# burchim/AVEC

Hardware: AMD Instinct MI355X
Metric: AV utterances/sec fwd+bwd (audio T=400, video 100x88x88) (higher is better)
Workload: dtype bf16

## Files before the change

avec_amd/csrc/gemm.hip:

```cpp
#include "gemm_dev.h"

template <typename T, int BM, int BN, int MODE, bool SRC_F32, bool A16>
__global__ __launch_bounds__(256, 2) void gemm_nt_kernel(GemmArgs g) {
  constexpr int VEC = Elt<T>::VEC;
  constexpr int KE = BKB / (int)sizeof(T);
  constexpr int NCA = BM * 8 / 256, NCB = BN * 8 / 256;
  constexpr int MT = BM / 64, NT = BN / 64;
  constexpr int TILE = (BM + BN) * LDS_ROW;
  extern __shared__ __attribute__((aligned(16))) char smem[];
  const int tid = threadIdx.x, lane = tid & 63, wave = tid >> 6;
  const int wm = wave >> 1, wn = wave & 1;
  const long long m0 = (long long)blockIdx.x * BM; const int n0 = blockIdx.y * BN;
  const int kc = (tid & 7) * VEC;
  const int r0 = tid >> 3;

  RowInfo ra[NCA]; RowInfo rb[NCB];
  RowSrc ws; ws.ptr = g.W; ws.ld = g.ldw; ws.step = 0; ws.rows_out = ws.rows_in = 1;
#pragma unroll
  for (int i = 0; i < NCA; ++i) ra[i] = row_info<MODE>(g.a, m0 + r0 + i * 32, g.M);
#pragma unroll
  for (int i = 0; i < NCB; ++i) rb[i] = row_info<MODE_PLAIN>(ws, n0 + r0 + i * 32, g.N);

  f32x16 acc[MT][NT];
#pragma unroll
// ... 738 lines not shown
    for (int j = 0; j < NT; ++j)
#pragma unroll
      for (int r = 0; r < 16; ++r) acc[i][j][r] = 0.f;
  const int KT = (g.K + KE - 1) / KE;
  constexpr int LPT = NCA + NCB;
#define AVEC_WAIT_VM(n) asm volatile("s_waitcnt vmcnt(%0)" ::"n"(n) : "memory")
#pragma unroll
  for (int st = 0; st < STAGES - 1; ++st) if (st < KT) issue(st, st);
  for (int kt = 0; kt < KT; ++kt) {
    const int newer = min(STAGES - 2, KT - 1 - kt);
    if (STAGES <= 2 || newer <= 0) AVEC_WAIT_VM(0);
    else if (newer == 1) AVEC_WAIT_VM(LPT);
    else AVEC_WAIT_VM(2 * LPT);
    __builtin_amdgcn_s_barrier();
    asm volatile("" ::: "memory");
    if (kt + STAGES - 1 < KT) issue(kt + STAGES - 1, (kt + STAGES - 1) % STAGES);
    const char* As = smem + (kt % STAGES) * TILE; const char* Bs = As + BM * RB;
#pragma unroll
    for (int s2 = 0; s2 < 2; ++s2) {
      chunk16 fa[MT][2], fb[NT][2];
#pragma unroll
      for (int i = 0; i < MT; ++i)
#pragma unroll
        for (int h = 0; h < 2; ++h) fa[i][h] = *(const chunk16*)(As + offa[i] + (((4 * s2 + 2 * gsel + h) ^ swa[i]) << 4));
#pragma unroll
      for (int j = 0; j < NT; ++j)
#pragma unroll
        for (int h = 0; h < 2; ++h) fb[j][h] = *(const chunk16*)(Bs + offb[j] + (((4 * s2 + 2 * gsel + h) ^ swb[j]) << 4));
      asm volatile("" ::: "memory");
#pragma unroll
      for (int i = 0; i < MT; ++i) {
        const i32x8 a = {(int)fa[i][0].w[0], (int)fa[i][0].w[1], (int)fa[i][0].w[2], (int)fa[i][0].w[3], (int)fa[i][1].w[0], (int)fa[i][1].w[1], (int)fa[i][1].w[2], (int)fa[i][1].w[3]};
#pragma unroll
        for (int j = 0; j < NT; ++j) {
          const i32x8 b = {(int)fb[j][0].w[0], (int)fb[j][0].w[1], (int)fb[j][0].w[2], (int)fb[j][0].w[3], (int)fb[j][1].w[0], (int)fb[j][1].w[1], (int)fb[j][1].w[2], (int)fb[j][1].w[3]};
          acc[i][j] = __builtin_amdgcn_mfma_scale_f32_32x32x64_f8f6f4(a, b, acc[i][j], 0, 0, 0, 127, 0, 127);
        }
      }
    }
  }
#undef AVEC_WAIT_VM
  const float sc = (fmaxf(*amax_a, 1e-20f) * (1.0f / 448.0f)) * (fmaxf(*amax_w, 1e-20f) * (1.0f / 448.0f));
#pragma unroll
  for (int i = 0; i < MT; ++i)
#pragma unroll
    for (int j = 0; j < NT; ++j)
#pragma unroll
      for (int r = 0; r < 16; ++r) acc[i][j][r] *= sc;
  __syncthreads();
  nt_epilogue<T, BM, BN, MT, NT>(g, acc, smem, m0, n0, tid, lane, wm, wn);
}

struct TnArgs { const void* P; long long ldp; RowSrc q; float* O; void* Oact; long long ldo; long long M; int I, J, Iq, Jq; int m_per_block; float* pcs;
                int split, nb_inner, xcd_map, q_ohw, q_mg, q_nwrap; long long sPo, sPi, sQo, sQi, sOo, sOi; };

__device__ __forceinline__ int tn_swz(int col) { return (((col >> 2) ^ (col >> 3) ^ (col >> 4)) & 1) << 4; }

template <typename T>
__device__ __forceinline__ void store_transposed(char* S, int col0, int p, const chunk16& c0, const chunk16& c1) {
  constexpr int VEC = Elt<T>::VEC;
  if (sizeof(T) == 4) {
#pragma unroll
    for (int e = 0; e < VEC; ++e) *(uint32_t*)(S + (col0 + e) * LDS_ROW + ((p ^ tn_swz(col0 + e)) << 2)) = c0.w[e];
  } else {
#pragma unroll
    for (int e = 0; e < VEC; ++e) {
      const uint32_t w = (e & 1) ? __builtin_amdgcn_perm(c1.w[e >> 1], c0.w[e >> 1], 0x07060302u) : __builtin_amdgcn_perm(c1.w[e >> 1], c0.w[e >> 1], 0x05040100u);
      *(uint32_t*)(S + (col0 + e) * LDS_ROW + ((p ^ tn_swz(col0 + e)) << 2)) = w;
    }
  }
}

template <typename T, int BM, int BN, int MT, int NT>
__device__ __forceinline__ void mma_tile_swz(const char* As, const char* Bs, int wm, int wn, int lane, f32x16 (&acc)[MT][NT]) {
  int offa[MT], offb[NT], lowa[MT], lowb[NT];
#pragma unroll
  for (int i = 0; i < MT; ++i) { const int row = wm * (BM / 2) + i * 32 + (lane & 31); offa[i] = row * LDS_ROW; lowa[i] = ((lane >> 5) * 16) ^ (tn_swz(row) << 2); }
#pragma unroll
  for (int j = 0; j < NT; ++j) { const int row = wn * (BN / 2) + j * 32 + (lane & 31); offb[j] = row * LDS_ROW; lowb[j] = ((lane >> 5) * 16) ^ (tn_swz(row) << 2); }
#pragma unroll
  for (int kk = 0; kk < 4; ++kk) {
    chunk16 fa[MT], fb[NT];
#pragma unroll
    for (int i = 0; i < MT; ++i) fa[i] = *(const chunk16*)(As + offa[i] + (lowa[i] ^ (kk * 32)));
#pragma unroll
    for (int j = 0; j < NT; ++j) fb[j] = *(const chunk16*)(Bs + offb[j] + (lowb[j] ^ (kk * 32)));
#pragma unroll
    for (int i = 0; i < MT; ++i)
#pragma unroll
      for (int j = 0; j < NT; ++j) Mma<T>::run(fa[i], fb[j], acc[i][j]);
  }
}

template <typename T, int BI, int BJ, int MODE, bool Q_F32, bool A16>
__device__ __forceinline__ void gemm_tn_body(TnArgs g, const int bx, const int by, const int bz) {
  constexpr int VEC = Elt<T>::VEC;
  constexpr int RPT = sizeof(T) == 2 ? 2 : 1;
  constexpr int KE = 32 * RPT;
  constexpr int CPR_I = BI / VEC, CPR_J = BJ / VEC;
  constexpr int NTI = 32 * CPR_I / 256, NTJ = 32 * CPR_J / 256;
  constexpr int MT = BI / 64, NT = BJ / 64;
  constexpr int TILE = (BI + BJ) * LDS_ROW;
  constexpr bool Q_CONV = (MODE == MODE_CONV_FWD);
  extern __shared__ __attribute__((aligned(16))) char smem[];
  const int tid = threadIdx.x, lane = tid & 63, wave = tid >> 6;
  const int wm = wave >> 1, wn = wave & 1;
  const int i0 = bx * BI, j0 = by * BJ;
// ... 215 lines not shown
  }
  constexpr int CS_RF = 64 / (CPI * 4), CS_N = (KT / 4) / (4 * CS_RF);
  const bool do_cs = g.pcs != nullptr && by == 0;
  const int cs_pc = lane % CPI, cs_r4 = (lane / CPI) & 3, cs_rs = lane / (CPI * 4);
  float cs[8] = {0.f, 0.f, 0.f, 0.f, 0.f, 0.f, 0.f, 0.f};
  constexpr int LPT = NLI + NLJ;
#define AVEC_WAIT_VM(n) asm volatile("s_waitcnt vmcnt(%0)" ::"n"(n) : "memory")
  const int KTN = (int)((me - mb + KT - 1) / KT);
#pragma unroll
  for (int st = 0; st < STAGES - 1; ++st) if (st < KTN) issue(mb + (long long)st * KT, st);
  for (int kt = 0; kt < KTN; ++kt) {
    const int newer = min(STAGES - 2, KTN - 1 - kt);
    if (STAGES <= 2 || newer <= 0) AVEC_WAIT_VM(0);
    else if (newer == 1) AVEC_WAIT_VM(LPT);
    else AVEC_WAIT_VM(2 * LPT);
    __builtin_amdgcn_s_barrier();
    asm volatile("" ::: "memory");
    if (kt + STAGES - 1 < KTN) issue(mb + (long long)(kt + STAGES - 1) * KT, (kt + STAGES - 1) % STAGES);
    const char* S = smem + (kt % STAGES) * TILE;
    if (do_cs) {
#pragma unroll
      for (int n = 0; n < CS_N; ++n) {
        const int m = cs_r4 + 4 * (wave * CS_RF + cs_rs + 4 * CS_RF * n);
        const chunk16 c = *(const chunk16*)(S + m * (BI * 2) + (cs_pc << 4));
#pragma unroll
        for (int e = 0; e < 4; ++e) { cs[2 * e] += __uint_as_float(c.w[e] << 16); cs[2 * e + 1] += __uint_as_float(c.w[e] & 0xffff0000u); }
      }
    }
#pragma unroll
    for (int kk = 0; kk < KT / 16; ++kk) {
      chunk16 fa[MTI], fb[MTJ];
#pragma unroll
      for (int i = 0; i < MTI; ++i) fa[i] = tr_read8(S + offa[i][0] + kk * 16 * BI * 2, S + offa[i][1] + kk * 16 * BI * 2);
#pragma unroll
      for (int j = 0; j < MTJ; ++j) fb[j] = tr_read8(S + offb[j][0] + kk * 16 * BJ * 2, S + offb[j][1] + kk * 16 * BJ * 2);
#pragma unroll
      for (int i = 0; i < MTI; ++i)
#pragma unroll
        for (int j = 0; j < MTJ; ++j) Mma<T>::run(fa[i], fb[j], acc[i][j]);
    }
  }
#undef AVEC_WAIT_VM
  if (do_cs) {
    float* red = (float*)smem;
    __syncthreads();
    if (tid < BI) red[tid] = 0.f;
    __syncthreads();
    const int cl = (cs_pc ^ tr_swz<BI>(cs_r4)) << 3;
#pragma unroll
    for (int e = 0; e < 8; ++e) atomicAdd(red + cl + e, cs[e]);
    __syncthreads();
    if (tid < BI && i0 + tid < g.I) atomicAdd(g.pcs + i0 + tid, red[tid]);
  }
#pragma unroll
  for (int j = 0; j < MTJ; ++j) {
    const int col = j0 + wj * (BJ / 2) + j * 32 + (lane & 31);
    if (col >= g.J) continue;
#pragma unroll
    for (int i = 0; i < MTI; ++i)
#pragma unroll
      for (int r = 0; r < 16; ++r) {
        const int row = i0 + wi * (BI / 2) + i * 32 + (r & 3) + 8 * (r >> 2) + 4 * (lane >> 5);
        if (row < g.I) atomicAdd(Op + (long long)row * g.ldo + col, acc[i][j][r]);
      }
  }
}

template <int BI, int BJ, int MODE, int STAGES, bool Q32 = false, int KT = 64>
__global__ __launch_bounds__(256, 2) void gemm_tn_tr_kernel(TnArgs g) {
  if (g.xcd_map) {
    int l = xcd_logical(blockIdx.x + gridDim.x * (blockIdx.y + gridDim.y * blockIdx.z), gridDim.x * gridDim.y * gridDim.z);
    const int bx = l % gridDim.x; l /= gridDim.x;
    tn_tr_body<BI, BJ, MODE, STAGES, Q32, KT>(g, bx, l % gridDim.y, l / gridDim.y);
  } else tn_tr_body<BI, BJ, MODE, STAGES, Q32, KT>(g, blockIdx.x, blockIdx.y, blockIdx.z);
}

struct TnItem { const void* P; const void* Q; float* O; float* pcs; int ldp, ldq, ldo, M, I, J, Iq, Jq, m_per_block, split, gx, gy, rows_out, rows_in, step, first; };
struct TnGroup { TnItem it[AVEC_TN_GROUP_MAX]; int n, total, xcd_map; };
template <int BT, int STG = 2, int KT = 32>
__global__ __launch_bounds__(256, 2) void gemm_tn_tr_grouped_kernel(TnGroup grp) {
  const int w = grp.xcd_map ? xcd_logical(blockIdx.x, grp.total) : (int)blockIdx.x;
  int lo = 0, hi = grp.n - 1;
  while (lo < hi) { const int mid = (lo + hi + 1) >> 1; if (grp.it[mid].first <= w) lo = mid; else hi = mid - 1; }
  const TnItem& t = grp.it[lo];
  TnArgs g; g.P = t.P; g.ldp = t.ldp; g.q.ptr = t.Q; g.q.ld = t.ldq; g.q.rows_out = t.rows_out; g.q.rows_in = t.rows_in; g.q.step = t.step;
  g.q.H = g.q.W = g.q.C = g.q.KH = g.q.KW = g.q.stride = g.q.pad = g.q.OH = g.q.OW = 0;
  g.O = t.O; g.Oact = nullptr; g.ldo = t.ldo; g.M = t.M; g.I = t.I; g.J = t.J; g.Iq = t.Iq; g.Jq = t.Jq; g.m_per_block = t.m_per_block; g.pcs = t.pcs;
  g.split = t.split; g.nb_inner = 1; g.xcd_map = 0; g.q_ohw = 1; g.q_mg = 0; g.q_nwrap = 0; g.sPo = g.sPi = g.sQo = g.sQi = g.sOo = g.sOi = 0;
  int l = w - t.first; const int bx = l % t.gx; l /= t.gx; const int by = l % t.gy; const int bz = l / t.gy;
  tn_tr_body<BT, BT, MODE_PLAIN, STG, false, KT>(g, bx, by, bz);
}

#include <stdint.h>
#include <stdlib.h>
#include <string.h>
static RowSrc make_src(const void* ptr, const avec_rows_t* d) {
  RowSrc s; s.ptr = ptr; s.ld = d->ld; s.rows_out = d->rows_out; s.rows_in = d->rows_in; s.step = d->step;
  s.H = d->H; s.W = d->W; s.C = d->C; s.KH = d->KH; s.KW = d->KW; s.stride = d->stride; s.pad = d->pad; s.OH = d->OH; s.OW = d->OW;
  return s;
}

template <typename K> static int want_lds(K kern, size_t bytes) {
  static const void* done[256]; static int ndone = 0;
  for (int i = 0; i < ndone; ++i) if (done[i] == (const void*)kern) return 0;
  hipError_t e = hipFuncSetAttribute((const void*)kern, hipFuncAttributeMaxDynamicSharedMemorySize, (int)bytes);
  if (e != hipSuccess) { avec_set_error("hipFuncSetAttribute failed: %s", hipGetErrorString(e)); return (int)e; }
  if (ndone < 256) done[ndone++] = (const void*)kern;
  return 0;
}

static bool aligned16(const void* p) { return (((uintptr_t)p) & 15) == 0; }
static bool epi_tr_ok(const GemmArgs& g) {
  static const bool off = getenv("AVEC_NO_EPI_TR") != nullptr;
  const Epi& e = g.e;
  return !off && !e.out_f32 && !e.out_pre && !e.bias && e.act == 0 && !(e.drop_p > 0.f) && !e.dact && !e.colsum && !e.bnb_y && g.N % 8 == 0 &&
         e.ldo % 8 == 0 && aligned16(e.out) && (!e.res || (e.res_act && e.ldres % 8 == 0 && aligned16(e.res)));
}

static bool plain_tr_ok(const GemmArgs& g) {
  static const bool off = getenv("AVEC_NO_PLAIN_TR") != nullptr || getenv("AVEC_NO_EPI_TR") != nullptr;
  const Epi& e = g.e;
  const long long ob = e.out_f32 ? 4 : 2;
  return !off && !e.colsum && !e.stats && !e.bnb_y && g.N % 8 == 0 && g.N >= 8 && aligned16(e.out) && (e.ldo * ob) % 16 == 0 &&
         (!e.out_pre || (aligned16(e.out_pre) && e.ldpre % 8 == 0)) && (!e.bias || aligned16(e.bias)) && (!e.dact || (aligned16(e.dact_z) && e.ldz % 8 == 0)) &&
         (!e.res || (aligned16(e.res) && (e.ldres * (e.res_act ? 2 : 4)) % 16 == 0));
}

template <typename T, int BM, int BN>
static int launch_nt_mode(const GemmArgs& g_in, int mode, int src_f32, hipStream_t st) {
  GemmArgs g = g_in;
  dim3 grid((unsigned)((g.M + BM - 1) / BM), (unsigned)((g.N + BN - 1) / BN));
  size_t lds = (size_t)2 * (BM + BN) * LDS_ROW;
  constexpr int VEC = Elt<T>::VEC;
  const bool f32src = src_f32 && sizeof(T) == 2;
  const bool a16 = aligned16(g.a.ptr) && aligned16(g.W) && g.K % VEC == 0 && g.ldw % VEC == 0 &&
                   (mode != MODE_PLAIN || (g.a.ld % (f32src ? 4 : VEC) == 0));
  static const bool use_glds_ = true;
  static const bool no_ktail = false;
  const bool plain_any = sizeof(T) == 2 && mode == MODE_PLAIN && !f32src && use_glds_ && !no_ktail && (g.K % 8 == 0 || g.K % 8 == 4) && g.K >= 8 && g.ldw >= g.K && g.a.ld >= g.K &&
                         g.a.step <= 1;
  g.ktail = (plain_any && g.K % 8 == 4) ? 4 : 0;
// ... 147 lines not shown
    static const bool no_perm = getenv("AVEC_NO_PERM2") != nullptr;
    if (!no_perm && dtype == AVEC_BF16 && g.fast_conv && a_mode == MODE_CONV_BWD && a_rows->stride == 2 && M == imgs * (long long)a_rows->H * a_rows->W) {
      g.perm2 = 1; g.pImgs = imgs;
    }
  }
  Epi& e = g.e;
  e.out = ep->out; e.ldo = ep->ldo; e.out_f32 = ep->out_f32; e.out_pre = ep->out_pre; e.ldpre = ep->ldpre; e.bias = ep->bias;
  e.act = ep->act; e.drop_p = ep->drop_p; e.rng = (const unsigned long long*)ep->rng; e.stream = ep->rng_stream;
  e.res = ep->res; e.ldres = ep->ldres; e.alpha = ep->alpha; e.res_act = ep->res_act; e.dact_z = ep->dact_z; e.ldz = ep->ldz; e.dact = ep->dact;
  e.colsum = ep->colsum; e.stats = ep->stats;
  e.bnb_y = ep->bnb_y; e.ldby = ep->ldby; e.bnb_ss = ep->bnb_ss; e.bnb_mask = ep->bnb_mask; e.res_cls0 = ep->res_cls0; e.res_mask = ep->res_mask;
  AVEC_CHECK_ARG(!e.res_mask || (dtype == AVEC_BF16 && !a_f32 && a_mode != AVEC_ROWS_PLAIN && e.res && e.res_act && !e.res_cls0 && e.ldres % 8 == 0),
                 "gemm_nt: res_mask needs a bf16 convolution product with a bf16 residual whose rows are whole 8-element pieces");
  AVEC_CHECK_ARG(!e.res_cls0 || (g.perm2 && e.res), "gemm_nt: res_cls0 needs a bf16 stride-2 backward-data product that runs in parity-class order");
  AVEC_CHECK_ARG(!e.bnb_y || (e.stats && N % 4 == 0 && !(e.ldo & 3) && !(e.ldby & 3) && !(e.ldres & 3) && !(e.ldz & 3) && !(e.ldpre & 3) && (!e.bnb_mask || e.bnb_ss) && (e.bnb_mask || e.dact == 2 || e.dact == 0)),
                 "gemm_nt: the BatchNorm-backward fusion needs stats, N %% 4 == 0 and row strides that are multiples of 4");
  AVEC_CHECK_ARG(!(e.drop_p > 0.f) || e.rng, "gemm_nt: dropout without rng state");
  int r = 1;
  if (dtype == AVEC_BF16 && !a_f32 && a_mode != AVEC_ROWS_PLAIN) r = launch_conv_shift(g, a_mode, stream);
  if (r == 1 && dtype == AVEC_BF16 && !a_f32 && a_mode != AVEC_ROWS_PLAIN) r = avec_launch_conv_s2(g, a_mode, stream);
  if (r == 1) r = (dtype == AVEC_BF16) ? launch_nt<bf16>(g, a_mode, a_f32, stream) : launch_nt<float>(g, a_mode, a_f32, stream);
  if (r) return r;
  AVEC_LAUNCH_CHECK();
  return 0;
}


extern "C" int avec_gemm_nt_fp8(const void* A, long long lda, const void* W, long long ldw, long long M, int N, int K,
                                const float* amax_a, const float* amax_w, const avec_epilogue_t* ep, hipStream_t stream) {
  AVEC_CHECK_ARG(A && W && ep && ep->out && amax_a && amax_w, "gemm_nt_fp8: null pointer");
  AVEC_CHECK_ARG(M > 0 && N > 0 && K > 0 && K % 16 == 0 && lda % 16 == 0 && ldw % 16 == 0 && aligned16(A) && aligned16(W),
                 "gemm_nt_fp8: M=%lld N=%d K=%d lda=%lld ldw=%lld: K and the row strides must be multiples of 16 bytes, operands 16-byte aligned", M, N, K, lda, ldw);
  GemmArgs g; memset(&g, 0, sizeof(g));
  g.a.ptr = A; g.a.ld = lda; g.W = W; g.ldw = ldw; g.M = M; g.N = N; g.K = K;
  Epi& e = g.e;
  e.out = ep->out; e.ldo = ep->ldo; e.out_f32 = ep->out_f32; e.out_pre = ep->out_pre; e.ldpre = ep->ldpre; e.bias = ep->bias;
  e.act = ep->act; e.drop_p = ep->drop_p; e.rng = (const unsigned long long*)ep->rng; e.stream = ep->rng_stream;
  e.res = ep->res; e.ldres = ep->ldres; e.alpha = ep->alpha; e.res_act = ep->res_act; e.dact_z = ep->dact_z; e.ldz = ep->ldz; e.dact = ep->dact;
  e.colsum = ep->colsum; e.stats = ep->stats;
  AVEC_CHECK_ARG(!(e.drop_p > 0.f) || e.rng, "gemm_nt_fp8: dropout without rng state");
#define F8(BM, BN, S_) do { dim3 grid((unsigned)((M + BM - 1) / BM), (unsigned)((N + BN - 1) / BN)); \
    const size_t ring = (size_t)S_ * (BM + BN) * 128, epi = (size_t)64 * (BN + 4) * 4 + 10 * BN * 4; const size_t lds = ring > epi ? ring : epi; \
    if (int r = want_lds(gemm_nt_fp8_kernel<BM, BN, S_>, lds)) return r; \
    hipLaunchKernelGGL((gemm_nt_fp8_kernel<BM, BN, S_>), grid, dim3(256), lds, stream, g, amax_a, amax_w); } while (0)
  const long long t128 = ((M + 127) / 128) * ((N + 127) / 128);
  if (N > 64 && t128 >= 384) F8(128, 128, 2);
  else if (((M + 127) / 128) * ((N + 63) / 64) >= 384) F8(128, 64, 2);
  else F8(64, 64, 4);
#undef F8
  AVEC_LAUNCH_CHECK();
  return 0;
}

static thread_local TnMulti* tn_collect = nullptr;
template <typename T, int BI, int BJ>
static int launch_tn_tile(TnArgs g, int mode, int q_f32, int nbatch, hipStream_t st) {
  constexpr int KE = BKB / (int)sizeof(T);
  int tiles = ((g.I + BI - 1) / BI) * ((g.J + BJ - 1) / BJ) * nbatch;
  long long ksteps = (g.M + KE - 1) / KE;
  static const long long wg_env = getenv("AVEC_TN_WGS") ? atoll(getenv("AVEC_TN_WGS")) : 0;
  const long long wg_target = wg_env > 0 ? wg_env : (mode != MODE_PLAIN ? 896 : 512);
  long long split = (wg_target + tiles - 1) / tiles; if (split > ksteps / 4) split = ksteps / 4; if (split < 1 || g.Oact) split = 1;
  long long per = ((ksteps + split - 1) / split) * KE;
  split = (g.M + per - 1) / per;
  g.m_per_block = (int)per; g.split = (int)split;
  dim3 grid((g.I + BI - 1) / BI, (g.J + BJ - 1) / BJ, (unsigned)(split * nbatch));
  size_t lds = (size_t)2 * (BI + BJ) * LDS_ROW;
  constexpr int VEC = Elt<T>::VEC;
  const bool f32src = q_f32 && sizeof(T) == 2;
  const bool a16 = nbatch == 1 && aligned16(g.P) && aligned16(g.q.ptr) && g.Iq % VEC == 0 && g.Jq % VEC == 0 && g.ldp % VEC == 0 &&
                   (mode != MODE_PLAIN || (g.q.ld % (f32src ? 4 : VEC) == 0));
  if (sizeof(T) == 2 && a16 && !f32src && !g.Oact && (mode == MODE_PLAIN || g.q_mg != 0)) {
    static const bool use_tr = true;
    if (use_tr) {
      static const int kt_env = getenv("AVEC_TN_KT") ? atoi(getenv("AVEC_TN_KT")) : 32;
      const long long q_elems = mode == MODE_PLAIN ? 0 : ((g.M + (long long)g.q.OH * g.q.OW - 1) / ((long long)g.q.OH * g.q.OW) + 1) * g.q.H * g.q.W * g.q.C;
      const bool q32 = q_elems < (1ll << 31);
#define LT(MODE, Q32, KT_) do { const size_t l2 = (size_t)2 * KT_ * (BI + BJ) * 2; g.q_nwrap = (KT_ + g.q_ohw - 1) / g.q_ohw; avec_note_kernel("gemm_tn_tr_kernel<%d,%d,%d,2,%d,%d>", BI, BJ, MODE, (int)Q32, KT_); if (int r = want_lds(gemm_tn_tr_kernel<BI, BJ, MODE, 2, Q32, KT_>, l2)) return r; \
        hipLaunchKernelGGL((gemm_tn_tr_kernel<BI, BJ, MODE, 2, Q32, KT_>), grid, dim3(256), l2, st, g); return 0; } while (0)
#define LK(KT_) do { if (mode == MODE_PLAIN) LT(MODE_PLAIN, false, KT_); else if (q32) LT(MODE_CONV_FWD, true, KT_); else LT(MODE_CONV_FWD, false, KT_); } while (0)
      if (kt_env == 64) LK(64); else LK(32);
#undef LK
#undef LT
    }
  }
  if (g.pcs) {
    static const bool side_wgrad = false;
    if (int r = colsum_launch(sizeof(T) == 2 ? AVEC_BF16 : AVEC_F32, g.P, g.ldp, g.pcs, g.M, g.I, !side_wgrad, st)) return r;
  }
#define L(MODE, F, A) do { avec_note_kernel("gemm_tn_kernel<%s,%d,%d,%d,%d,%d>", (sizeof(T) == 2 ? "bf16" : "float"), BI, BJ, MODE, (int)F, (int)A); if (int r = want_lds(gemm_tn_kernel<T, BI, BJ, MODE, F, A>, lds)) return r; hipLaunchKernelGGL((gemm_tn_kernel<T, BI, BJ, MODE, F, A>), grid, dim3(256), lds, st, g); } while (0)
  if (tn_collect && sizeof(T) == 2 && BI == 64 && BJ == 64 && mode == MODE_PLAIN && !f32src && !a16 && !g.pcs && tn_collect->n < AVEC_TN_MULTI_MAX) {
    TnMulti& m = *tn_collect; const int k = m.n++;
    m.g[k] = g; m.gx[k] = (int)grid.x; m.gy[k] = (int)grid.y; m.first[k + 1] = m.first[k] + (int)(grid.x * grid.y * grid.z);
    return 0;
  }
  if (mode == MODE_PLAIN) {
    if (f32src) { if (a16) L(MODE_PLAIN, true, true); else L(MODE_PLAIN, true, false); }
    else { if (a16) L(MODE_PLAIN, false, true); else L(MODE_PLAIN, false, false); }
  } else { if (a16) L(MODE_CONV_FWD, false, true); else L(MODE_CONV_FWD, false, false); }
#undef L
  return 0;
}

static int gemm_tn_impl(int dtype, const void* P, long long ldp, const void* Q, const avec_rows_t* q_rows, int q_mode, int q_f32,
                        float* O, void* Oact, long long ldo, long long M, int I, int J, int nb_outer, int nb_inner, const long long* strides, float* p_colsum, hipStream_t stream) {
  AVEC_CHECK_ARG(dtype == AVEC_F32 || dtype == AVEC_BF16, "gemm_tn: bad dtype %d", dtype);
  AVEC_CHECK_ARG(P && Q && (O || Oact) && q_rows, "gemm_tn: null pointer");
  AVEC_CHECK_ARG(M > 0 && I > 0 && J > 0 && nb_outer > 0 && nb_inner > 0, "gemm_tn: bad dims");
  AVEC_CHECK_ARG(q_mode == MODE_PLAIN || q_mode == MODE_CONV_FWD, "gemm_tn: bad q_mode %d", q_mode);
  const int vec = dtype == AVEC_BF16 ? 8 : 4;
  const int Jq = (q_mode == MODE_PLAIN && q_rows->ld >= (J + vec - 1) / vec * vec) ? (J + vec - 1) / vec * vec : J;
  const int Iq = (ldp >= (I + vec - 1) / vec * vec) ? (I + vec - 1) / vec * vec : I;
  AVEC_CHECK_ARG(Iq >= vec && Jq >= vec && (dtype == AVEC_F32 || (Iq % 2 == 0 && Jq % 2 == 0 && ldp % 2 == 0)), "gemm_tn: I=%d, J=%d: need >= %d and (bf16) even I, J, ldp", I, J, vec);
  AVEC_CHECK_ARG(q_mode != MODE_PLAIN || dtype == AVEC_F32 || q_rows->ld % 2 == 0, "gemm_tn: ldq must be even");
  AVEC_CHECK_ARG(q_mode == MODE_PLAIN || q_rows->C % vec == 0, "gemm_tn: conv C=%d must be a multiple of %d", q_rows->C, vec);
  AVEC_CHECK_ARG(!(q_f32 && dtype == AVEC_BF16) || Jq % 4 == 0, "gemm_tn: fp32-source staging needs J %% 4 == 0");
  TnArgs g; g.P = P; g.ldp = ldp; g.q = make_src(Q, q_rows); g.O = O; g.Oact = Oact; g.ldo = ldo; g.M = M; g.I = I; g.J = J; g.Iq = Iq; g.Jq = Jq; g.m_per_block = 0; g.pcs = p_colsum;
  g.split = 1; g.nb_inner = nb_inner;
  g.q_ohw = 1; g.q_mg = 0; g.q_nwrap = 0;
  if (q_mode != MODE_PLAIN && q_rows->OW > 0 && q_rows->OH > 0 && (long long)q_rows->OH * q_rows->OW <= 4096) {
    const int ohw = q_rows->OH * q_rows->OW; const unsigned mg = ((1u << 20) + (unsigned)q_rows->OW - 1u) / (unsigned)q_rows->OW;
    bool exact = true; for (int px = 0; px < ohw && exact; ++px) exact = (int)(((unsigned)px * mg) >> 20) == px / q_rows->OW;
    g.q_ohw = ohw; g.q_mg = exact ? (int)mg : 0;
  }
  { static const bool no_xcd = false; g.xcd_map = no_xcd ? 0 : 1; }
  g.sPo = strides ? strides[0] : 0; g.sPi = strides ? strides[1] : 0; g.sQo = strides ? strides[2] : 0; g.sQi = strides ? strides[3] : 0;
  g.sOo = strides ? strides[4] : 0; g.sOi = strides ? strides[5] : 0;
  if (dtype == AVEC_BF16 && strides) for (int i = 0; i < 2; ++i) AVEC_CHECK_ARG(strides[i] % 2 == 0, "gemm_tn: bf16 batch strides of P must be even");
  const int nbatch = nb_outer * nb_inner;
  bool big = (I >= 128 && J >= 128) && ((long long)((I + 127) / 128) * ((J + 127) / 128) * nbatch >= 48 || M >= 32768);
  int r;
  const bool wide = !big && I <= 64 && J >= 128 && M >= 32768 && dtype == AVEC_BF16 && !q_f32 && nbatch == 1 && aligned16(P) && aligned16(Q) && Iq % 8 == 0 && Jq % 8 == 0 &&
                    ldp % 8 == 0 && (q_mode != MODE_PLAIN || q_rows->ld % 8 == 0);
  if (dtype == AVEC_BF16) r = big ? launch_tn_tile<bf16, 128, 128>(g, q_mode, q_f32, nbatch, stream) : wide ? launch_tn_tile<bf16, 64, 128>(g, q_mode, q_f32, nbatch, stream)
                                                                                                    : launch_tn_tile<bf16, 64, 64>(g, q_mode, q_f32, nbatch, stream);
  else r = big ? launch_tn_tile<float, 128, 128>(g, q_mode, q_f32, nbatch, stream) : launch_tn_tile<float, 64, 64>(g, q_mode, q_f32, nbatch, stream);
  if (r) return r;
  AVEC_LAUNCH_CHECK();
  return 0;
}

extern "C" int avec_gemm_tn(int dtype, const void* P, long long ldp, const void* Q, const avec_rows_t* q_rows, int q_mode, int q_f32,
                            float* O, long long ldo, long long M, int I, int J, hipStream_t stream) {
  return gemm_tn_impl(dtype, P, ldp, Q, q_rows, q_mode, q_f32, O, nullptr, ldo, M, I, J, 1, 1, nullptr, nullptr, stream);
}
extern "C" int avec_gemm_tn_bias(int dtype, const void* P, long long ldp, const void* Q, const avec_rows_t* q_rows, int q_mode, int q_f32,
                                 float* O, long long ldo, float* p_colsum, long long M, int I, int J, hipStream_t stream) {
  AVEC_CHECK_ARG(!p_colsum || (I % 4 == 0 && ldp % 4 == 0), "gemm_tn_bias: column sums need I %% 4 == 0 and ldp %% 4 == 0");
  return gemm_tn_impl(dtype, P, ldp, Q, q_rows, q_mode, q_f32, O, nullptr, ldo, M, I, J, 1, 1, nullptr, p_colsum, stream);
}

extern "C" int avec_gemm_tn_batched(int dtype, const void* P, long long ldp, const void* Q, long long ldq, float* O, long long ldo, long long M, int I, int J,
                                    int nb_outer, int nb_inner, const long long* strides6, hipStream_t stream) {
  avec_rows_t rows = {}; rows.ld = ldq;
  AVEC_CHECK_ARG(strides6, "gemm_tn_batched: null strides");
  return gemm_tn_impl(dtype, P, ldp, Q, &rows, MODE_PLAIN, 0, O, nullptr, ldo, M, I, J, nb_outer, nb_inner, strides6, nullptr, stream);
}
extern "C" int avec_gemm_tn_batched_store(int dtype, const void* P, long long ldp, const void* Q, long long ldq, void* O_act, long long ldo, long long M, int I, int J,
                                          int nb_outer, int nb_inner, const long long* strides6, hipStream_t stream) {
  avec_rows_t rows = {}; rows.ld = ldq;
  AVEC_CHECK_ARG(strides6 && O_act, "gemm_tn_batched_store: null pointer");
  return gemm_tn_impl(dtype, P, ldp, Q, &rows, MODE_PLAIN, 0, nullptr, O_act, ldo, M, I, J, nb_outer, nb_inner, strides6, nullptr, stream);
}

extern "C" int avec_gemm_tn_batched_multi(int dtype, const avec_tn_batched_t* items, int n, hipStream_t stream) {
  AVEC_CHECK_ARG(items && n >= 1 && n <= AVEC_TN_MULTI_MAX, "gemm_tn_batched_multi: need 1..%d problems (got %d)", AVEC_TN_MULTI_MAX, n);
  static const bool off = false;
  TnMulti m; m.n = 0; m.first[0] = 0;
  if (!off) tn_collect = &m;
  int rc = 0;
  for (int k = 0; k < n && rc == 0; ++k) {
    const avec_tn_batched_t& t = items[k];
    avec_rows_t rows = {}; rows.ld = t.ldq;
    if (!t.strides6 || (!t.O && !t.O_act)) { avec_set_error("gemm_tn_batched_multi: problem %d: null pointer", k); rc = -1; break; }
    rc = gemm_tn_impl(dtype, t.P, t.ldp, t.Q, &rows, MODE_PLAIN, 0, t.O_act ? nullptr : t.O, t.O_act, t.ldo, t.M, t.I, t.J, t.nb_outer, t.nb_inner, t.strides6, nullptr, stream);
  }
  tn_collect = nullptr;
  if (rc) return rc;
  if (m.n > 0) {
    const size_t lds = (size_t)2 * (64 + 64) * LDS_ROW;
    avec_note_kernel("gemm_tn_multi_kernel<%d>", m.n);
    if (int r = want_lds(gemm_tn_multi_kernel, lds)) return r;
    hipLaunchKernelGGL(gemm_tn_multi_kernel, dim3((unsigned)m.first[m.n]), dim3(256), lds, stream, m);
    AVEC_LAUNCH_CHECK();
  }
  return 0;
}

static bool tn_item_ok(int dtype, const avec_tn_item_t& t) {
  if (dtype != AVEC_BF16 || !t.P || !t.Q || !t.O || t.M <= 0 || t.I <= 0 || t.J <= 0) return false;
  if (t.ldp < t.I || t.ldq < t.J) return false;
  if (t.p_colsum && (t.I % 4 || t.ldp % 4)) return false;
  return t.M < (1ll << 31) && t.ldp < (1ll << 31) && t.ldq < (1ll << 31) && t.ldo < (1ll << 31);
}
extern "C" int avec_gemm_tn_grouped_ok(int dtype, const avec_tn_item_t* item) { return item && tn_item_ok(dtype, *item) ? 1 : 0; }

extern "C" int avec_gemm_tn_grouped(int dtype, const avec_tn_item_t* items, int n, hipStream_t stream) {
  AVEC_CHECK_ARG(items && n > 0 && n <= AVEC_TN_GROUP_MAX, "gemm_tn_grouped: need 1..%d items (got %d)", AVEC_TN_GROUP_MAX, n);
  for (int k = 0; k < n; ++k) AVEC_CHECK_ARG(tn_item_ok(dtype, items[k]), "gemm_tn_grouped: item %d is not eligible (bf16 operands, row strides >= widths, bias sums need I %% 4 == 0)", k);
  static const int bt_env = 0;
  long long t128 = 0;
  for (int k = 0; k < n; ++k) t128 += (long long)((items[k].I + 127) / 128) * ((items[k].J + 127) / 128);
  const int BT = bt_env == 64 || bt_env == 128 ? bt_env : (t128 >= 96 ? 128 : 64);
  static const long long wg_env = 0;
  const long long wg_target = wg_env > 0 ? wg_env : 512;
  long long per = 256;
  for (long long cand = 8192; cand >= 256; cand -= 64) {
    long long wgs = 0;
    for (int k = 0; k < n; ++k) wgs += (long long)((items[k].I + BT - 1) / BT) * ((items[k].J + BT - 1) / BT) * ((items[k].M + cand - 1) / cand);
    if (wgs >= wg_target) { per = cand; break; }
  }
  TnGroup grp; grp.n = n;
  int first = 0;
  for (int k = 0; k < n; ++k) {
    const avec_tn_item_t& s = items[k]; TnItem& t = grp.it[k];
    t.P = s.P; t.Q = s.Q; t.O = s.O; t.pcs = s.p_colsum; t.ldp = (int)s.ldp; t.ldq = (int)s.ldq; t.ldo = (int)s.ldo; t.M = (int)s.M; t.I = s.I; t.J = s.J;
    t.Iq = (s.I + 7) / 8 * 8; t.Jq = (s.J + 7) / 8 * 8;
    t.rows_out = s.q_rows_out > 0 ? s.q_rows_out : 1; t.rows_in = s.q_rows_in > 0 ? s.q_rows_in : 1; t.step = s.q_step;
    long long mp = per; if (mp > s.M) mp = (s.M + 63) / 64 * 64;
    t.m_per_block = (int)mp; t.split = (int)((s.M + mp - 1) / mp);
    t.gx = (s.I + BT - 1) / BT; t.gy = (s.J + BT - 1) / BT; t.first = first;
    first += t.gx * t.gy * t.split;
  }
  grp.total = first;
  static const bool no_xcd = false;
  grp.xcd_map = no_xcd ? 0 : 1;
  static const int kt_env = 64;
  static const int stg_env = 2;
  const int KT = kt_env == 32 ? 32 : 64, STG = (stg_env == 4 && KT == 32) ? 4 : 2;
  const size_t lds = (size_t)STG * KT * (BT + BT) * 2;
  avec_note_kernel("gemm_tn_tr_grouped_kernel<%d,%d,%d>", BT, STG, KT);
#define TNG(BT_, S_, K_) do { if (BT == BT_ && STG == S_ && KT == K_) { if (int r = want_lds(gemm_tn_tr_grouped_kernel<BT_, S_, K_>, lds)) return r; \
    hipLaunchKernelGGL((gemm_tn_tr_grouped_kernel<BT_, S_, K_>), dim3((unsigned)first), dim3(256), lds, stream, grp); } } while (0)
  TNG(128, 2, 32); TNG(128, 2, 64); TNG(64, 2, 32); TNG(64, 2, 64); TNG(128, 4, 32); TNG(64, 4, 32);
#undef TNG
  AVEC_LAUNCH_CHECK();
  return 0;
}
```

avec_amd/csrc/vec.h:

```cpp
#pragma once
#include "common.h"
#include <cstdlib>

template <typename T> __device__ __forceinline__ void ld4(const T* p, float v[4]);
template <> __device__ __forceinline__ void ld4<float>(const float* p, float v[4]) { float4 t = *(const float4*)p; v[0] = t.x; v[1] = t.y; v[2] = t.z; v[3] = t.w; }
template <> __device__ __forceinline__ void ld4<bf16>(const bf16* p, float v[4]) {
  uint2 t = *(const uint2*)p;
  v[0] = __uint_as_float(t.x << 16); v[1] = __uint_as_float(t.x & 0xffff0000u);
  v[2] = __uint_as_float(t.y << 16); v[3] = __uint_as_float(t.y & 0xffff0000u);
}
template <typename T> __device__ __forceinline__ void st4(T* p, const float v[4]);
template <> __device__ __forceinline__ void st4<float>(float* p, const float v[4]) { *(float4*)p = make_float4(v[0], v[1], v[2], v[3]); }
template <> __device__ __forceinline__ void st4<bf16>(bf16* p, const float v[4]) {
  uint2 t; t.x = f32x2_to_bf16x2(v[0], v[1]);
  t.y = f32x2_to_bf16x2(v[2], v[3]);
  *(uint2*)p = t;
}

template <typename T> __device__ __forceinline__ void ld8(const T* p, float v[8]);
template <> __device__ __forceinline__ void ld8<float>(const float* p, float v[8]) { ld4<float>(p, v); ld4<float>(p + 4, v + 4); }
template <> __device__ __forceinline__ void ld8<bf16>(const bf16* p, float v[8]) {
  uint4 t = *(const uint4*)p; const uint32_t w[4] = {t.x, t.y, t.z, t.w};
#pragma unroll
  for (int k = 0; k < 4; ++k) { v[2 * k] = __uint_as_float(w[k] << 16); v[2 * k + 1] = __uint_as_float(w[k] & 0xffff0000u); }
}
template <typename T> __device__ __forceinline__ void st8(T* p, const float v[8]);
template <> __device__ __forceinline__ void st8<float>(float* p, const float v[8]) { st4<float>(p, v); st4<float>(p + 4, v + 4); }
template <> __device__ __forceinline__ void st8<bf16>(bf16* p, const float v[8]) {
  uint4 t;
  t.x = f32x2_to_bf16x2(v[0], v[1]); t.y = f32x2_to_bf16x2(v[2], v[3]);
  t.z = f32x2_to_bf16x2(v[4], v[5]); t.w = f32x2_to_bf16x2(v[6], v[7]);
  *(uint4*)p = t;
}

__device__ __forceinline__ void bf8_to_f32(const uint4& t, float v[8]) {
  const uint32_t w[4] = {t.x, t.y, t.z, t.w};
#pragma unroll
  for (int k = 0; k < 4; ++k) { v[2 * k] = __uint_as_float(w[k] << 16); v[2 * k + 1] = __uint_as_float(w[k] & 0xffff0000u); }
}
template <typename T> struct Raw8;
template <> struct Raw8<bf16> { uint4 t; __device__ __forceinline__ void load(const bf16* p) { t = *(const uint4*)p; } __device__ __forceinline__ void get(float v[8]) const { bf8_to_f32(t, v); } };
template <> struct Raw8<float> { float4 a, b; __device__ __forceinline__ void load(const float* p) { a = *(const float4*)p; b = *(const float4*)(p + 4); }
  __device__ __forceinline__ void get(float v[8]) const { v[0] = a.x; v[1] = a.y; v[2] = a.z; v[3] = a.w; v[4] = b.x; v[5] = b.y; v[6] = b.z; v[7] = b.w; } };
#define DISPATCH_T(dtype, ...) do { if ((dtype) == AVEC_BF16) { typedef bf16 T; __VA_ARGS__; } else { typedef float T; __VA_ARGS__; } } while (0)


struct ColWs { float* partial; };
ColWs avec_reduce_ws(size_t partial_floats, hipStream_t st);

__device__ __forceinline__ float* ws_slot(const ColWs& ws, unsigned colblock, unsigned slot, unsigned nslots, int ncols) {
  return ws.partial + ((size_t)colblock * nslots + slot) * ncols;
}
static constexpr int FIN_MAXNV = 20;
struct ColFin { const float* partial; float* dst[FIN_MAXNV]; int NV, W, C, nslots, dstride; };
__global__ __launch_bounds__(256) void col_finalize_kernel(ColFin f);
int colsum_launch(int dtype, const void* x, long long ld, float* out, long long M, int N, bool use_ws, hipStream_t st);
int col_finalize(const ColWs& ws, unsigned colblocks, unsigned nslots, int NV, int W, float* const* dst, int C, hipStream_t st, int dstride = 1);

template <int NV>
__device__ __forceinline__ void colreduce_atomic(float (&part)[NV][4], float* const (&dst)[NV], int col, int C, const ColWs& ws = ColWs{nullptr}) {
  __shared__ float red[8][32][4];
  const int tx = threadIdx.x & 31, ty = threadIdx.x >> 5;
  float* mine = ws.partial ? ws_slot(ws, blockIdx.x, blockIdx.y, gridDim.y, NV * 128) : nullptr;
#pragma unroll
  for (int n = 0; n < NV; ++n) {
    for (int e = 0; e < 4; ++e) red[ty][tx][e] = part[n][e];
    __syncthreads();
    if (ty == 0) {
      for (int e = 0; e < 4; ++e) {
        float s = 0.f;
        for (int y = 0; y < 8; ++y) s += red[y][tx][e];
        if (mine) mine[n * 128 + tx * 4 + e] = s;
        else if (col + e < C && dst[n]) atomicAdd(dst[n] + col + e, s);
      }
    }
    __syncthreads();
  }
}
static inline ColWs col_ws(dim3 grid, int NV, hipStream_t st) { return avec_reduce_ws((size_t)grid.x * grid.y * NV * 128, st); }
static inline long long col_ws_min_atomics() { return 16384; }
static inline ColWs col_ws_if(dim3 grid, int NV, int C, hipStream_t st) {
  const long long atomics = (long long)grid.y * NV * C;
  return atomics > col_ws_min_atomics() ? col_ws(grid, NV, st) : ColWs{nullptr};
}

static inline dim3 col_grid(long long M, int C) {
  unsigned gx = (unsigned)((C / 4 + 31) / 32);
  long long gy = (M + 63) / 64; long long cap = 2048 / gx; if (cap < 1) cap = 1; if (gy > cap) gy = cap; if (gy < 1) gy = 1;
  return dim3(gx, (unsigned)gy);
}

struct Col8 { int L, R, r, l; bool active; };
__device__ __forceinline__ Col8 col8_map(int C) {
  Col8 m; m.L = C >> 3; m.R = 256 / m.L; m.r = threadIdx.x / m.L; m.l = threadIdx.x - m.r * m.L; m.active = m.r < m.R; return m;
}
template <int NV>
__device__ __forceinline__ void colreduce8_atomic(float (&part)[NV][8], float* const (&dst)[NV], const Col8& m, const ColWs& ws = ColWs{nullptr}) {
  __shared__ float red8[NV * 8][256];
#pragma unroll
  for (int n = 0; n < NV; ++n)
#pragma unroll
    for (int e = 0; e < 8; ++e) red8[n * 8 + e][threadIdx.x] = m.active ? part[n][e] : 0.f;
  __syncthreads();
  const int C = m.L * 8;
  float* mine = ws.partial ? ws_slot(ws, 0, blockIdx.x, gridDim.x, NV * C) : nullptr;
  for (int o = threadIdx.x; o < NV * 8 * m.L; o += 256) {
    const int q = o / m.L, l = o - q * m.L; float s = 0.f;
    for (int rr = 0; rr < m.R; ++rr) s += red8[q][rr * m.L + l];
    if (mine) mine[(q >> 3) * C + l * 8 + (q & 7)] = s;
    else {
// ... 21 lines not shown
```

Measured before the change: 1844.

## Replace split-K atomic accumulation in TN weight-grad GEMMs with slab reduction

Split-K partial tiles from the TN (weight-gradient) GEMM kernels are now written to a workspace slab instead of being atomically added to the output. A new grouped tile-slab-sum kernel then reduces the partials deterministically and adds them into the output. Grouped items with no split and no output overlap get plain read-modify-write stores instead of atomics. The aim is to cut float atomic contention on output tiles, at the cost of extra workspace traffic and one more kernel launch.

Result: no change. 1829 (-0.8%).

```diff
diff --git a/avec_amd/csrc/gemm.hip b/avec_amd/csrc/gemm.hip
--- a/avec_amd/csrc/gemm.hip
+++ b/avec_amd/csrc/gemm.hip
@@ -814,7 +814,8 @@
 }
 
 struct TnArgs { const void* P; long long ldp; RowSrc q; float* O; void* Oact; long long ldo; long long M; int I, J, Iq, Jq; int m_per_block; float* pcs;
-                int split, nb_inner, xcd_map, q_ohw, q_mg, q_nwrap; long long sPo, sPi, sQo, sQi, sOo, sOi; };
+                int split, nb_inner, xcd_map, q_ohw, q_mg, q_nwrap; long long sPo, sPi, sQo, sQi, sOo, sOi;
+                float* slab; int slab_gx, own; };
 
 __device__ __forceinline__ int tn_swz(int col) { return (((col >> 2) ^ (col >> 3) ^ (col >> 4)) & 1) << 4; }
 
@@ -1136,6 +1137,17 @@
     __syncthreads();
     if (tid < BI && i0 + tid < g.I) atomicAdd(g.pcs + i0 + tid, red[tid]);
   }
+  if (g.slab) {
+    float* sp = g.slab + ((long long)(by * g.slab_gx + bx) * g.split + zs) * (BI * BJ) + wave * (MTI * MTJ * 1024) + lane * 4;
+#pragma unroll
+    for (int i = 0; i < MTI; ++i)
+#pragma unroll
+      for (int j = 0; j < MTJ; ++j)
+#pragma unroll
+        for (int q = 0; q < 4; ++q)
+          *(float4*)(sp + ((i * MTJ + j) * 4 + q) * 256) = make_float4(acc[i][j][4 * q], acc[i][j][4 * q + 1], acc[i][j][4 * q + 2], acc[i][j][4 * q + 3]);
+    return;
+  }
 #pragma unroll
   for (int j = 0; j < MTJ; ++j) {
     const int col = j0 + wj * (BJ / 2) + j * 32 + (lane & 31);
@@ -1145,9 +1157,43 @@
 #pragma unroll
       for (int r = 0; r < 16; ++r) {
         const int row = i0 + wi * (BI / 2) + i * 32 + (r & 3) + 8 * (r >> 2) + 4 * (lane >> 5);
-        if (row < g.I) atomicAdd(Op + (long long)row * g.ldo + col, acc[i][j][r]);
-      }
-  }
+        if (row < g.I) { float* o = Op + (long long)row * g.ldo + col; if (g.own) *o += acc[i][j][r]; else atomicAdd(o, acc[i][j][r]); }
+      }
+  }
+}
+
+__global__ __launch_bounds__(256) void tn_slab_sum_kernel(TsGroup grp) {
+  __shared__ float4 red[256];
+  const int w = blockIdx.x, tid = threadIdx.x;
+  int lo = 0, hi = grp.n - 1;
+  while (lo < hi) { const int mid = (lo + hi + 1) >> 1; if (grp.it[mid].first <= w) lo = mid; else hi = mid - 1; }
+  const TsItem& t = grp.it[lo];
+  const int BI = grp.BI, BJ = grp.BJ, sg = grp.sg, LP = 256 / sg, tile4 = BI * BJ / 4, CH = tile4 / LP;
+  const int l = w - t.first, tile = l / CH, idx4 = (l - tile * CH) * LP + (tid % LP), cls = tid / LP;
+  const float* sp = grp.slab + ((long long)t.tile0 + (long long)tile * t.split) * (BI * BJ) + idx4 * 4;
+  float4 a = make_float4(0.f, 0.f, 0.f, 0.f);
+  int s = cls;
+  for (; s + 3 * sg < t.split; s += 4 * sg) {
+    const float4 v0 = *(const float4*)(sp + (long long)s * (BI * BJ)), v1 = *(const float4*)(sp + (long long)(s + sg) * (BI * BJ));
+    const float4 v2 = *(const float4*)(sp + (long long)(s + 2 * sg) * (BI * BJ)), v3 = *(const float4*)(sp + (long long)(s + 3 * sg) * (BI * BJ));
+    a.x = (((a.x + v0.x) + v1.x) + v2.x) + v3.x; a.y = (((a.y + v0.y) + v1.y) + v2.y) + v3.y; a.z = (((a.z + v0.z) + v1.z) + v2.z) + v3.z; a.w = (((a.w + v0.w) + v1.w) + v2.w) + v3.w;
+  }
+  for (; s < t.split; s += sg) { const float4 v = *(const float4*)(sp + (long long)s * (BI * BJ)); a.x += v.x; a.y += v.y; a.z += v.z; a.w += v.w; }
+  if (sg > 1) {
+    red[tid] = a;
+    __syncthreads();
+    if (cls != 0) return;
+    for (int c = 1; c < sg; ++c) { const float4 v = red[c * LP + tid]; a.x += v.x; a.y += v.y; a.z += v.z; a.w += v.w; }
+  }
+  const int MTI = BI / 64, MTJ = BJ / 64, lane = idx4 & 63, q = (idx4 >> 6) & 3;
+  int u = idx4 >> 8; const int j = u % MTJ; u /= MTJ; const int i = u % MTI, wave = u / MTI;
+  const int bx = tile % t.gx, by = tile / t.gx;
+  const int row = bx * BI + (wave >> 1) * (BI / 2) + i * 32 + 8 * q + 4 * (lane >> 5), col = by * BJ + (wave & 1) * (BJ / 2) + j * 32 + (lane & 31);
+  if (col >= t.J) return;
+  float* o = t.O + (long long)row * t.ldo + col;
+  const float v[4] = {a.x, a.y, a.z, a.w};
+#pragma unroll
+  for (int e = 0; e < 4; ++e) if (row + e < t.I) o[(long long)e * t.ldo] += v[e];
 }
 
 template <int BI, int BJ, int MODE, int STAGES, bool Q32 = false, int KT = 64>
@@ -1159,8 +1205,8 @@
   } else tn_tr_body<BI, BJ, MODE, STAGES, Q32, KT>(g, blockIdx.x, blockIdx.y, blockIdx.z);
 }
 
-struct TnItem { const void* P; const void* Q; float* O; float* pcs; int ldp, ldq, ldo, M, I, J, Iq, Jq, m_per_block, split, gx, gy, rows_out, rows_in, step, first; };
-struct TnGroup { TnItem it[AVEC_TN_GROUP_MAX]; int n, total, xcd_map; };
+struct TnItem { const void* P; const void* Q; float* O; float* pcs; int ldp, ldq, ldo, M, I, J, Iq, Jq, m_per_block, split, gx, gy, rows_out, rows_in, step, first, slab0, own; };
+struct TnGroup { TnItem it[AVEC_TN_GROUP_MAX]; float* slab; int n, total, xcd_map; };
 template <int BT, int STG = 2, int KT = 32>
 __global__ __launch_bounds__(256, 2) void gemm_tn_tr_grouped_kernel(TnGroup grp) {
   const int w = grp.xcd_map ? xcd_logical(blockIdx.x, grp.total) : (int)blockIdx.x;
@@ -1171,6 +1217,7 @@
   g.q.H = g.q.W = g.q.C = g.q.KH = g.q.KW = g.q.stride = g.q.pad = g.q.OH = g.q.OW = 0;
   g.O = t.O; g.Oact = nullptr; g.ldo = t.ldo; g.M = t.M; g.I = t.I; g.J = t.J; g.Iq = t.Iq; g.Jq = t.Jq; g.m_per_block = t.m_per_block; g.pcs = t.pcs;
   g.split = t.split; g.nb_inner = 1; g.xcd_map = 0; g.q_ohw = 1; g.q_mg = 0; g.q_nwrap = 0; g.sPo = g.sPi = g.sQo = g.sQi = g.sOo = g.sOi = 0;
+  g.slab = t.slab0 >= 0 ? grp.slab + (long long)t.slab0 * (BT * BT) : nullptr; g.slab_gx = t.gx; g.own = t.own;
   int l = w - t.first; const int bx = l % t.gx; l /= t.gx; const int by = l % t.gy; const int bz = l / t.gy;
   tn_tr_body<BT, BT, MODE_PLAIN, STG, false, KT>(g, bx, by, bz);
 }
@@ -1424,6 +1471,19 @@
   return 0;
 }
 
+static int tn_slabs_on() { static const int on = getenv("AVEC_TN_SLABS") ? atoi(getenv("AVEC_TN_SLABS")) : 7; return on; }
+static int g_tn_last[4];
+extern "C" int avec_tn_last_launch(int* out4) { for (int i = 0; i < 4; ++i) out4[i] = g_tn_last[i]; return 0; }
+int tile_slab_sum(TsGroup& grp, hipStream_t st) {
+  int smax = 1, first = 0;
+  for (int k = 0; k < grp.n; ++k) if (grp.it[k].split > smax) smax = grp.it[k].split;
+  grp.sg = smax >= 16 ? 4 : 1;
+  const int ch = grp.BI * grp.BJ / 4 / (256 / grp.sg);
+  for (int k = 0; k < grp.n; ++k) { TsItem& t = grp.it[k]; t.first = first; first += t.gx * ((t.J + grp.BJ - 1) / grp.BJ) * ch; }
+  hipLaunchKernelGGL(tn_slab_sum_kernel, dim3((unsigned)first), dim3(256), 0, st, grp);
+  return 0;
+}
+
 static thread_local TnMulti* tn_collect = nullptr;
 template <typename T, int BI, int BJ>
 static int launch_tn_tile(TnArgs g, int mode, int q_f32, int nbatch, hipStream_t st) {
@@ -1448,8 +1508,18 @@
       static const int kt_env = getenv("AVEC_TN_KT") ? atoi(getenv("AVEC_TN_KT")) : 32;
       const long long q_elems = mode == MODE_PLAIN ? 0 : ((g.M + (long long)g.q.OH * g.q.OW - 1) / ((long long)g.q.OH * g.q.OW) + 1) * g.q.H * g.q.W * g.q.C;
       const bool q32 = q_elems < (1ll << 31);
+      TsGroup ts; ts.n = 0;
+      if (split > 1 && nbatch == 1 && (tn_slabs_on() & 4)) {
+        const ColWs ws = avec_reduce_ws((size_t)tiles * (size_t)split * BI * BJ, st);
+        if (ws.partial) {
+          g.slab = ws.partial; g.slab_gx = (int)grid.x;
+          ts.n = 1; ts.slab = ws.partial; ts.BI = BI; ts.BJ = BJ;
+          TsItem& t = ts.it[0]; t.O = g.O; t.ldo = (int)g.ldo; t.I = g.I; t.J = g.J; t.gx = (int)grid.x; t.split = (int)split; t.tile0 = 0;
+        }
+      }
+      g_tn_last[0] = (int)split; g_tn_last[1] = ts.n; g_tn_last[2] = 0; g_tn_last[3] = 1 - ts.n;
 #define LT(MODE, Q32, KT_) do { const size_t l2 = (size_t)2 * KT_ * (BI + BJ) * 2; g.q_nwrap = (KT_ + g.q_ohw - 1) / g.q_ohw; avec_note_kernel("gemm_tn_tr_kernel<%d,%d,%d,2,%d,%d>", BI, BJ, MODE, (int)Q32, KT_); if (int r = want_lds(gemm_tn_tr_kernel<BI, BJ, MODE, 2, Q32, KT_>, l2)) return r; \
-        hipLaunchKernelGGL((gemm_tn_tr_kernel<BI, BJ, MODE, 2, Q32, KT_>), grid, dim3(256), l2, st, g); return 0; } while (0)
+        hipLaunchKernelGGL((gemm_tn_tr_kernel<BI, BJ, MODE, 2, Q32, KT_>), grid, dim3(256), l2, st, g); return ts.n ? tile_slab_sum(ts, st) : 0; } while (0)
 #define LK(KT_) do { if (mode == MODE_PLAIN) LT(MODE_PLAIN, false, KT_); else if (q32) LT(MODE_CONV_FWD, true, KT_); else LT(MODE_CONV_FWD, false, KT_); } while (0)
       if (kt_env == 64) LK(64); else LK(32);
 #undef LK
@@ -1488,7 +1558,7 @@
   AVEC_CHECK_ARG(q_mode == MODE_PLAIN || q_rows->C % vec == 0, "gemm_tn: conv C=%d must be a multiple of %d", q_rows->C, vec);
   AVEC_CHECK_ARG(!(q_f32 && dtype == AVEC_BF16) || Jq % 4 == 0, "gemm_tn: fp32-source staging needs J %% 4 == 0");
   TnArgs g; g.P = P; g.ldp = ldp; g.q = make_src(Q, q_rows); g.O = O; g.Oact = Oact; g.ldo = ldo; g.M = M; g.I = I; g.J = J; g.Iq = Iq; g.Jq = Jq; g.m_per_block = 0; g.pcs = p_colsum;
-  g.split = 1; g.nb_inner = nb_inner;
+  g.split = 1; g.nb_inner = nb_inner; g.slab = nullptr; g.slab_gx = 0; g.own = 0;
   g.q_ohw = 1; g.q_mg = 0; g.q_nwrap = 0;
   if (q_mode != MODE_PLAIN && q_rows->OW > 0 && q_rows->OH > 0 && (long long)q_rows->OH * q_rows->OW <= 4096) {
     const int ohw = q_rows->OH * q_rows->OW; const unsigned mg = ((1u << 20) + (unsigned)q_rows->OW - 1u) / (unsigned)q_rows->OW;
@@ -1574,7 +1644,7 @@
   long long t128 = 0;
   for (int k = 0; k < n; ++k) t128 += (long long)((items[k].I + 127) / 128) * ((items[k].J + 127) / 128);
   const int BT = bt_env == 64 || bt_env == 128 ? bt_env : (t128 >= 96 ? 128 : 64);
-  static const long long wg_env = 0;
+  static const long long wg_env = getenv("AVEC_TNG_WGS") ? atoll(getenv("AVEC_TNG_WGS")) : 0;
   const long long wg_target = wg_env > 0 ? wg_env : 512;
   long long per = 256;
   for (long long cand = 8192; cand >= 256; cand -= 64) {
@@ -1591,10 +1661,32 @@
     t.rows_out = s.q_rows_out > 0 ? s.q_rows_out : 1; t.rows_in = s.q_rows_in > 0 ? s.q_rows_in : 1; t.step = s.q_step;
     long long mp = per; if (mp > s.M) mp = (s.M + 63) / 64 * 64;
     t.m_per_block = (int)mp; t.split = (int)((s.M + mp - 1) / mp);
-    t.gx = (s.I + BT - 1) / BT; t.gy = (s.J + BT - 1) / BT; t.first = first;
+    t.gx = (s.I + BT - 1) / BT; t.gy = (s.J + BT - 1) / BT; t.first = first; t.slab0 = -1; t.own = 0;
     first += t.gx * t.gy * t.split;
   }
-  grp.total = first;
+  grp.total = first; grp.slab = nullptr;
+  TsGroup ts; ts.n = 0; ts.BI = ts.BJ = BT;
+  int smax = 1, n_own = 0;
+  if (tn_slabs_on()) {
+    long long slabs = 0;
+    for (int k = 0; k < n; ++k) {
+      TnItem& t = grp.it[k]; if (t.split > smax) smax = t.split;
+      const float* lo = t.O; const float* hi = t.O + (long long)(t.I - 1) * t.ldo + t.J;
+      bool alone = true;
+      for (int m = 0; m < n && alone; ++m) if (m != k) { const TnItem& u = grp.it[m]; alone = !(u.O < hi && lo < u.O + (long long)(u.I - 1) * u.ldo + u.J); }
+      if (!alone) continue;
+      if (t.split == 1) { if (tn_slabs_on() & 2) { t.own = 1; ++n_own; } }
+      else if (tn_slabs_on() & 1) { t.slab0 = (int)slabs; slabs += (long long)t.gx * t.gy * t.split; }
+    }
+    const ColWs ws = slabs > 0 && slabs < (1 << 24) ? avec_reduce_ws((size_t)slabs * BT * BT, stream) : ColWs{nullptr};
+    for (int k = 0; k < n; ++k) {
+      TnItem& t = grp.it[k]; if (t.slab0 < 0) continue;
+      if (!ws.partial) { t.slab0 = -1; continue; }
+      TsItem& q = ts.it[ts.n++]; q.O = t.O; q.ldo = t.ldo; q.I = t.I; q.J = t.J; q.gx = t.gx; q.split = t.split; q.tile0 = t.slab0;
+    }
+    grp.slab = ws.partial; ts.slab = ws.partial;
+  }
+  g_tn_last[0] = smax; g_tn_last[1] = ts.n; g_tn_last[2] = n_own; g_tn_last[3] = n - ts.n - n_own;
   static const bool no_xcd = false;
   grp.xcd_map = no_xcd ? 0 : 1;
   static const int kt_env = 64;
@@ -1606,6 +1698,7 @@
     hipLaunchKernelGGL((gemm_tn_tr_grouped_kernel<BT_, S_, K_>), dim3((unsigned)first), dim3(256), lds, stream, grp); } } while (0)
   TNG(128, 2, 32); TNG(128, 2, 64); TNG(64, 2, 32); TNG(64, 2, 64); TNG(128, 4, 32); TNG(64, 4, 32);
 #undef TNG
+  if (ts.n) tile_slab_sum(ts, stream);
   AVEC_LAUNCH_CHECK();
   return 0;
 }
diff --git a/avec_amd/csrc/vec.h b/avec_amd/csrc/vec.h
--- a/avec_amd/csrc/vec.h
+++ b/avec_amd/csrc/vec.h
@@ -56,6 +56,12 @@
 __global__ __launch_bounds__(256) void col_finalize_kernel(ColFin f);
 int colsum_launch(int dtype, const void* x, long long ld, float* out, long long M, int N, bool use_ws, hipStream_t st);
 int col_finalize(const ColWs& ws, unsigned colblocks, unsigned nslots, int NV, int W, float* const* dst, int C, hipStream_t st, int dstride = 1);
+
+static constexpr int TS_MAX = 32;
+struct TsItem { float* O; int ldo, I, J, gx, split, tile0, first; };
+struct TsGroup { TsItem it[TS_MAX]; const float* slab; int n, BI, BJ, sg; };
+__global__ __launch_bounds__(256) void tn_slab_sum_kernel(TsGroup grp);
+int tile_slab_sum(TsGroup& grp, hipStream_t st);
 
 template <int NV>
 __device__ __forceinline__ void colreduce_atomic(float (&part)[NV][4], float* const (&dst)[NV], int col, int C, const ColWs& ws = ColWs{nullptr}) {
```
